# ThinkLib/Sail

Hardware: AMD Instinct MI355X
Metric: Msamples/s (paths x bounces) at 1920x1080 Cornell box (higher is better)
Workload: dtype f32; 1 GPU; cornell_box_readme_C2; width=1920, height=1080, bounces=8, spp=1024, launch_spp=1024, partition=tiles64x1, processes=one

## Files before the change

include/sail_hip.h:

```cpp
#ifndef SAIL_HIP_H
#define SAIL_HIP_H
#include <stddef.h>
#include <stdint.h>

#ifdef __cplusplus
extern "C" {
#endif

#define SAIL_ABI_VERSION 4

enum sail_status {
  SAIL_OK = 0,
  SAIL_E_INVALID = -1,
  SAIL_E_HIP = -2,
  SAIL_E_OOM = -3,
  SAIL_E_STATE = -4,
  SAIL_E_RCCL = -5,
  SAIL_E_NODEVICE = -6
};

enum sail_flags {
  SAIL_FLAG_AOV = 1u << 0,
  SAIL_FLAG_SEGMENT_COUNT = 1u << 1
};
// ... 133 lines not shown
  SAIL_JIT_MODE_FLAT = 0,
  SAIL_JIT_MODE_CULL = 1,
  SAIL_JIT_MODE_ROOM = 2
};
int sail_jit_compile(const sail_plugins* plugins, int mode, const int32_t* row_types, int rows, void* code,
                     size_t* bytes);
enum sail_kernel_jit_state {
  SAIL_KERNEL_JIT_NONE = 0,
  SAIL_KERNEL_JIT_PENDING = 1,
  SAIL_KERNEL_JIT_READY = 2,
  SAIL_KERNEL_JIT_FAILED = 3
};
typedef struct sail_kernel_info {
  char name[64];
  uint64_t build_id;
  int jit_state;
  int jit_from_cache;
  double jit_compile_ms;
  uint64_t jit_build_id;
  char jit_error[256];
} sail_kernel_info;
int sail_get_kernel_info(sail_ctx* ctx, sail_kernel_info* out);
int sail_kernel_ready(sail_ctx* ctx, int timeout_ms, int* ready);
int sail_set_jit_cache(const char* dir);
int sail_jit_prebuild(const float* objects, int n, const float* texparams, int tn, const float* lights, int ln,
                      const sail_plugins* plugins, const char* arch, const char* dir, int* built);

int sail_camera(const double eye[3], const double center[3], const double up[3], double fovy, double aspect,
                double znear, double zfar, double mvp_rowmajor[16]);
int sail_jitter_inverse(const double mvp_rowmajor[16], double jx, double jy, int width, int height, float inv_colmajor[16]);
int sail_schedule(const double mvp_rowmajor[16], int width, int height, int k0, int spp, float* inv_colmajor, float* seeds);

int sail_prim_bounds(const float* objects, int n, int tn, float* out_minmax);

int sail_comm_unique_id(char id[128]);
int sail_comm_init(sail_ctx* ctx, const char id[128], int nranks, int rank);
int sail_reduce(sail_ctx* ctx, int root);
int sail_accum_device_ptr(sail_ctx* ctx, void** ptr, size_t* bytes);
int sail_partition_tiles(int width, int height, int rank, int world, int* out_xywh, int capacity);
typedef struct sail_reduce_plan {
  int receives;
  int tiles;
  int aov_owner;
  int send_own_aovs;
  uint64_t samples;
} sail_reduce_plan;
int sail_plan_reduce(int width, int height, int rank, int world, int mode, uint64_t k, int root, sail_reduce_plan* out);
int sail_plan_keep(int width, int height, int rank, int world, int mode, const float* sums, float* out);
int sail_plan_load_part(uint64_t* missing, uint64_t* k, int parts, int part, uint64_t k_part);

int sail_math_probe(int fn, const float* x, const float* y, float* out, int count);
int sail_abi_version(void);
int sail_kernel_name(sail_ctx* ctx, char* name, int len);
int sail_filter_ms(sail_ctx* ctx, double* ms);

#ifdef __cplusplus
}
#endif
#endif
```

sail_amd/capi.py:

```python
from __future__ import annotations

import ctypes
import os
from typing import Optional, Sequence

import numpy as np

_HERE = os.path.dirname(os.path.abspath(__file__))
LIB_PATH = os.environ.get("SAIL_HIP_LIB") or os.path.join(_HERE, "lib", "libsail_hip.so")

SAIL_OK = 0
FLAG_AOV = 1
FLAG_SEGMENT_COUNT = 2
ACCUM_SUM, ACCUM_MIX, ACCUM_COMPAT8 = 0, 1, 2
PART_TILES, PART_SAMPLES = 0, 1
FILTER_COLOR, FILTER_GAMMA, FILTER_TONEMAPPING, FILTER_WINDOW = 0, 1, 2, 3
FILTER_WAVELET, FILTER_NORMAL, FILTER_POSITION = 4, 5, 6
DEBUG_CULL_MIN_PRIMS, DEBUG_FORCE_GENERIC, DEBUG_CULL_FMA, DEBUG_SAMPLE_GROUPS, DEBUG_FORCE_RCCL = 1, 2, 3, 4, 5
DEBUG_WAVEFRONT = 6
DEBUG_GROUP_ROUNDS = 7
DEBUG_CULL_GROUP_ROUNDS = 8
DEBUG_JIT = 9
DEBUG_JIT_WAIT = 10
DEBUG_JIT_NT = 12
DEBUG_JIT_NS = 11
KERNEL_JIT_NONE, KERNEL_JIT_PENDING, KERNEL_JIT_READY, KERNEL_JIT_FAILED = 0, 1, 2, 3
JIT_MODE_FLAT, JIT_MODE_CULL, JIT_MODE_ROOM = 0, 1, 2
DEBUG_DEFAULTS: dict = {}

EXPORTS = (
    "sail_create", "sail_create_multi", "sail_set_debug", "sail_destroy", "sail_last_error", "sail_device_count", "sail_device_info", "sail_set_scene",
    "sail_update_objects", "sail_set_accum_mode", "sail_set_partition", "sail_set_launch_samples",
    "sail_render", "sail_render_schedule", "sail_reset", "sail_sync", "sail_readback", "sail_read_accum",
    "sail_filter", "sail_get_stats", "sail_camera", "sail_jitter_inverse", "sail_schedule",
    "sail_comm_unique_id", "sail_comm_init", "sail_reduce", "sail_accum_device_ptr", "sail_partition_tiles",
    "sail_prim_bounds", "sail_math_probe", "sail_pick", "sail_kernel_name", "sail_filter_ms",
    "sail_abi_version", "sail_accum_parts", "sail_save_accum", "sail_load_accum", "sail_jit_compile",
    "sail_get_kernel_info", "sail_kernel_ready", "sail_set_jit_cache", "sail_jit_prebuild",
    "sail_plan_reduce", "sail_plan_keep", "sail_plan_load_part",
    "sail_noise_mark", "sail_noise_estimate", "sail_plan_until", "sail_render_until",
    "sail_denoise_defaults", "sail_denoise",
    "sail_temporal_defaults", "sail_gbuffer", "sail_temporal_begin", "sail_temporal_resolve", "sail_temporal_read",
    "sail_temporal_load_history",
)


class SailError(RuntimeError):
    pass


class Plugins(ctypes.Structure):
    _fields_ = [("shape_mask", ctypes.c_uint32), ("material_mask", ctypes.c_uint32),
                ("texture_mask", ctypes.c_uint32), ("light_mask", ctypes.c_uint32)]


class Stats(ctypes.Structure):
    _fields_ = [("samples", ctypes.c_uint64), ("segments", ctypes.c_uint64),
                ("nominal_segments", ctypes.c_uint64), ("kernel_ms", ctypes.c_double),
                ("last_launch_ms", ctypes.c_double), ("launches", ctypes.c_uint32)]


class KernelInfo(ctypes.Structure):
    _fields_ = [("name", ctypes.c_char * 64), ("build_id", ctypes.c_uint64), ("jit_state", ctypes.c_int),
                ("jit_from_cache", ctypes.c_int), ("jit_compile_ms", ctypes.c_double), ("jit_build_id", ctypes.c_uint64),
                ("jit_error", ctypes.c_char * 256)]


class ReducePlan(ctypes.Structure):
    _fields_ = [("receives", ctypes.c_int), ("tiles", ctypes.c_int), ("aov_owner", ctypes.c_int),
                ("send_own_aovs", ctypes.c_int), ("samples", ctypes.c_uint64)]


# ... 61 lines not shown
    vp = ctypes.c_void_p
    sig = {
        "sail_create": (ctypes.c_int, [ctypes.POINTER(vp), ctypes.c_int, ctypes.c_int, ctypes.c_int, ctypes.c_uint32]),
        "sail_create_multi": (ctypes.c_int, [ctypes.POINTER(vp), ctypes.c_int, ctypes.c_int, ctypes.POINTER(ctypes.c_int),
                                             ctypes.c_int, ctypes.c_uint32]),
        "sail_set_debug": (ctypes.c_int, [vp, ctypes.c_int, ctypes.c_int]),
        "sail_destroy": (None, [vp]),
        "sail_last_error": (ctypes.c_char_p, [vp]),
        "sail_device_count": (ctypes.c_int, [ctypes.POINTER(ctypes.c_int)]),
        "sail_device_info": (ctypes.c_int, [ctypes.c_int, ctypes.POINTER(ctypes.c_int), ctypes.POINTER(ctypes.c_int)]),
        "sail_set_scene": (ctypes.c_int, [vp, f32p, ctypes.c_int, f32p, ctypes.c_int, f32p, ctypes.c_int, ctypes.POINTER(Plugins)]),
        "sail_update_objects": (ctypes.c_int, [vp, f32p, ctypes.c_int]),
        "sail_set_accum_mode": (ctypes.c_int, [vp, ctypes.c_int]),
        "sail_set_partition": (ctypes.c_int, [vp, ctypes.c_int, ctypes.c_int, ctypes.c_int]),
        "sail_set_launch_samples": (ctypes.c_int, [vp, ctypes.c_int]),
        "sail_render": (ctypes.c_int, [vp, f32p, f32p, ctypes.c_float, ctypes.c_int]),
        "sail_render_schedule": (ctypes.c_int, [vp, f32p, f32p, f32p, ctypes.c_int, ctypes.c_int]),
        "sail_reset": (ctypes.c_int, [vp]),
        "sail_sync": (ctypes.c_int, [vp]),
        "sail_readback": (ctypes.c_int, [vp, f32p, f32p, f32p]),
        "sail_read_accum": (ctypes.c_int, [vp, f32p]),
        "sail_filter": (ctypes.c_int, [vp, ctypes.c_int, f32p, ctypes.c_float, ctypes.c_float, ctypes.c_float, f32p, ctypes.POINTER(ctypes.c_uint8)]),
        "sail_get_stats": (ctypes.c_int, [vp, ctypes.POINTER(Stats)]),
        "sail_camera": (ctypes.c_int, [f64p, f64p, f64p, ctypes.c_double, ctypes.c_double, ctypes.c_double, ctypes.c_double, f64p]),
        "sail_jitter_inverse": (ctypes.c_int, [f64p, ctypes.c_double, ctypes.c_double, ctypes.c_int, ctypes.c_int, f32p]),
        "sail_schedule": (ctypes.c_int, [f64p, ctypes.c_int, ctypes.c_int, ctypes.c_int, ctypes.c_int, f32p, f32p]),
        "sail_comm_unique_id": (ctypes.c_int, [ctypes.c_char_p]),
        "sail_comm_init": (ctypes.c_int, [vp, ctypes.c_char_p, ctypes.c_int, ctypes.c_int]),
        "sail_reduce": (ctypes.c_int, [vp, ctypes.c_int]),
        "sail_accum_device_ptr": (ctypes.c_int, [vp, ctypes.POINTER(vp), ctypes.POINTER(ctypes.c_size_t)]),
        "sail_partition_tiles": (ctypes.c_int, [ctypes.c_int, ctypes.c_int, ctypes.c_int, ctypes.c_int,
                                                 ctypes.POINTER(ctypes.c_int), ctypes.c_int]),
        "sail_prim_bounds": (ctypes.c_int, [f32p, ctypes.c_int, ctypes.c_int, f32p]),
        "sail_math_probe": (ctypes.c_int, [ctypes.c_int, f32p, f32p, f32p, ctypes.c_int]),
        "sail_abi_version": (ctypes.c_int, []),
        "sail_pick": (ctypes.c_int, [vp, f32p, ctypes.c_int, ctypes.POINTER(ctypes.c_int32), f32p]),
        "sail_kernel_name": (ctypes.c_int, [vp, ctypes.c_char_p, ctypes.c_int]),
        "sail_filter_ms": (ctypes.c_int, [vp, f64p]),
        "sail_accum_parts": (ctypes.c_int, [vp, ctypes.POINTER(ctypes.c_int)]),
        "sail_save_accum": (ctypes.c_int, [vp, ctypes.c_int, f32p, ctypes.POINTER(ctypes.c_uint64)]),
        "sail_load_accum": (ctypes.c_int, [vp, ctypes.c_int, f32p, ctypes.c_uint64]),
        "sail_jit_compile": (ctypes.c_int, [ctypes.POINTER(Plugins), ctypes.c_int, ctypes.POINTER(ctypes.c_int32), ctypes.c_int,
                                            vp, ctypes.POINTER(ctypes.c_size_t)]),
        "sail_get_kernel_info": (ctypes.c_int, [vp, ctypes.POINTER(KernelInfo)]),
        "sail_kernel_ready": (ctypes.c_int, [vp, ctypes.c_int, ctypes.POINTER(ctypes.c_int)]),
        "sail_set_jit_cache": (ctypes.c_int, [ctypes.c_char_p]),
        "sail_jit_prebuild": (ctypes.c_int, [f32p, ctypes.c_int, f32p, ctypes.c_int, f32p, ctypes.c_int, ctypes.POINTER(Plugins),
                                             ctypes.c_char_p, ctypes.c_char_p, ctypes.POINTER(ctypes.c_int)]),
        "sail_plan_reduce": (ctypes.c_int, [ctypes.c_int, ctypes.c_int, ctypes.c_int, ctypes.c_int, ctypes.c_int,
                                            ctypes.c_uint64, ctypes.c_int, ctypes.POINTER(ReducePlan)]),
        "sail_plan_keep": (ctypes.c_int, [ctypes.c_int, ctypes.c_int, ctypes.c_int, ctypes.c_int, ctypes.c_int, f32p, f32p]),
        "sail_plan_load_part": (ctypes.c_int, [ctypes.POINTER(ctypes.c_uint64), ctypes.POINTER(ctypes.c_uint64), ctypes.c_int,
                                               ctypes.c_int, ctypes.c_uint64]),
        "sail_noise_mark": (ctypes.c_int, [vp]),
        "sail_noise_estimate": (ctypes.c_int, [vp, ctypes.POINTER(NoiseInfo), f32p, f32p, ctypes.c_int]),
        "sail_plan_until": (ctypes.c_int, [ctypes.c_uint64, ctypes.c_uint64, ctypes.c_uint64, ctypes.POINTER(ctypes.c_uint64)]),
        "sail_render_until": (ctypes.c_int, [vp, f64p, f32p, ctypes.c_int, ctypes.c_double, ctypes.c_uint64, ctypes.c_uint64,
                                             ctypes.POINTER(NoiseInfo), ctypes.POINTER(ctypes.c_int),
                                             ctypes.POINTER(UntilStep), ctypes.c_int, ctypes.POINTER(ctypes.c_int)]),
        "sail_denoise_defaults": (ctypes.c_int, [ctypes.POINTER(DenoiseParams)]),
        "sail_denoise": (ctypes.c_int, [vp, ctypes.POINTER(DenoiseParams), f32p, f32p, ctypes.POINTER(ctypes.c_uint8),
                                        ctypes.POINTER(DenoiseInfo)]),
        "sail_temporal_defaults": (ctypes.c_int, [ctypes.POINTER(TemporalParams)]),
        "sail_gbuffer": (ctypes.c_int, [vp, f64p, f32p, f32p, ctypes.POINTER(ctypes.c_int32), f32p, f32p]),
        "sail_temporal_begin": (ctypes.c_int, [vp, f64p, f32p, ctypes.POINTER(TemporalParams), ctypes.POINTER(TemporalInfo)]),
        "sail_temporal_resolve": (ctypes.c_int, [vp, ctypes.POINTER(TemporalParams), f32p, ctypes.POINTER(ctypes.c_uint8),
# ... 135 lines not shown
    if rc:
        raise SailError(f"sail_temporal_defaults: {rc}")
    return {"cap": p.cap, "pos_tol": p.pos_tol, "display": p.display, "gamma_c": p.gamma_c}


def _temporal_params(params: Optional[dict], who: str):
    if params is None:
        return None
    d = temporal_defaults()
    unknown = set(params) - set(d)
    if unknown:
        raise SailError(f"{who}: unknown parameters {sorted(unknown)}")
    d.update(params)
    return TemporalParams(float(d["cap"]), float(d["pos_tol"]), int(d["display"]), float(d["gamma_c"]))


def _temporal_dict(i: TemporalInfo) -> dict:
    return {"k": int(i.k), "hit_pixels": int(i.hit_pixels), "history_pixels": int(i.history_pixels),
            "nonfinite": int(i.nonfinite), "kernel_ms": i.kernel_ms, "pass_ms": [i.pass_ms[j] for j in range(3)]}


def prim_bounds(objects, n: int, tn: int) -> np.ndarray:
    lib = load()
    rows = _f32(objects).reshape(-1)
    if rows.size < 18 * n:
        raise SailError("prim_bounds: fewer than 18 floats per row")
    out = np.zeros((max(n, 1), 6), dtype=np.float32)
    rc = lib.sail_prim_bounds(_ptr(rows), n, tn, _ptr(out))
    if rc:
        raise SailError(f"sail_prim_bounds: {rc}")
    return out[:n].reshape(n, 2, 3)


def math_probe(fn: int, x: np.ndarray, y: Optional[np.ndarray] = None) -> np.ndarray:
    lib = load()
    x = _f32(x)
    y = _f32(np.zeros_like(x) if y is None else y)
    out = np.zeros_like(x)
    rc = lib.sail_math_probe(fn, _ptr(x), _ptr(y), _ptr(out), int(x.size))
    if rc:
        raise SailError(f"sail_math_probe: {lib.sail_last_error(None).decode()}")
    return out


def device_count() -> int:
    lib = load()
    n = ctypes.c_int(0)
    lib.sail_device_count(ctypes.byref(n))
    return n.value


def device_info(device: int = 0):
    lib = load()
    cus, khz = ctypes.c_int(0), ctypes.c_int(0)
    if lib.sail_device_info(device, ctypes.byref(cus), ctypes.byref(khz)) != 0:
        raise SailError(f"sail_device_info({device}) failed")
    return cus.value, khz.value * 1e3


def set_jit_cache(path: Optional[str]):
    load().sail_set_jit_cache(None if path is None else path.encode())


def jit_prebuild(sc: dict, arch: str = "gfx950", cache_dir: Optional[str] = None) -> bool:
    lib = load()
    o, t, l = _f32(sc["objects"]), _f32(sc["texparams"]), _f32(sc["lights"])
# ... 313 lines not shown
```

sail_amd/csrc/sail_capi.cpp:

```cpp
#include <hip/hip_runtime.h>
#include <dlfcn.h>
#include <math.h>
#include <algorithm>
#include <cmath>
#include <stdarg.h>
#include <stdio.h>
#include <stdlib.h>
#include <string.h>
#include <string>
#include <vector>
#include "../../include/sail_hip.h"
#include "sail_device.h"

hipError_t sail_launch_trace(const SailTraceArgs& A, int blocks, hipStream_t s);
#include "sail_jit.h"
hipError_t sail_launch_filter(const SailFilterArgs& A, hipStream_t s);
hipError_t sail_launch_accum(const SailTraceArgs& A, int blocks, hipStream_t s);
hipError_t sail_launch_math(int fn, const float* x, const float* y, float* out, int count);
hipError_t sail_launch_sum(const SailSumArgs& A, hipStream_t s);
hipError_t sail_launch_negzero_unowned(float4* a, float4* b, int W, int H, int rank, int world, hipStream_t s);
hipError_t sail_launch_wavefront(const SailTraceArgs& A, const SailWfState& S, hipStream_t s);
hipError_t sail_launch_pick(const SailPrim* prims, int n, const float* rays, int count, int32_t* index, float* t,
                            hipStream_t s);
#include "sail_noise.h"
// ... 76 lines not shown
    out[2] = at(px, y);
  }
};

}

struct SceneBox { double lo[3], hi[3]; double diag; };

struct sail_ctx {
  int device = 0, W = 0, H = 0;
  uint32_t flags = 0;
  hipStream_t stream = nullptr;
  float4* accum = nullptr;
  float4* aovN = nullptr;
  float4* aovP = nullptr;
  float4* filterOut = nullptr;
  uint8_t* filterOut8 = nullptr;
  unsigned long long* segCounter = nullptr;
  SailPrim* prims = nullptr;
  float* tp = nullptr;
  float* lt = nullptr;
  int32_t* lightObjRow = nullptr;
  SailSample* samples = nullptr;
  int samplesCap = 0;
  int samplesPos = 0;
  SailSample* samplesPinned = nullptr;
  std::vector<SailSample> hostSamples;
  std::vector<float> objectsRows;
  std::vector<float> tpRows;
  int n = 0, tn = 0, ln = 0;
  sail_plugins plugins{};
  bool haveScene = false;
  int shadowAnyHit = 0;
  std::vector<unsigned long long> typeMasksHost;
  int cullMinPrims = 8;
  int lastGroups = 1;
  bool lastWavefront = false;
  int flatGroupRounds = 36;
  int cullGroupRounds = 64;
  int cullFma = 1;
  double primExtent = INFINITY;
  SceneBox scene{};
  int forceGeneric = 0;
  int forceGroups = 0;
  int wavefront = 0;
  int jit = 27;
  bool jitHave = false;
  SailJitSpec jitSpec;
  int jitMode = 0;
  int jitState = SAIL_KERNEL_JIT_NONE;
  SailJitKernel jitK;
  std::string jitError;
  int jitWait = 0;
  int jitNt = 0;
  int jitNs = 0;
  bool lastJit = false;
  int lastJitMode = 0;
  uint64_t lastBuildId = 0;
  std::vector<int> primTypes;
  float4* wf = nullptr;
  size_t wfSlots = 0;
  int numCUs = 256;
  float* stage = nullptr;
  size_t stageBytes = 0;
  int accumMode = SAIL_ACCUM_SUM;
  int rank = 0, world = 1, partMode = SAIL_PART_TILES;
// ... 375 lines not shown
}

double primExtent(const std::vector<SailPrim>& prims) {
  double m = 0.0;
  for (const SailPrim& p : prims)
    for (int k = 18; k < 24; k++) m = fmax(m, std::isfinite(p.a[k]) ? fabs((double)p.a[k]) : INFINITY);
  return m;
}

bool cullFmaOk(const sail_ctx* c) {
  const double e = fmax(fmax(fabs(c->eyeCache[0]), fabs(c->eyeCache[1])), fabs(c->eyeCache[2]));
  return c->cullFma && fmax(c->primExtent, e) < 4096.0;
}

int eyeNearScene(const sail_ctx* c) {
  double d2 = 0.0;
  for (int k = 0; k < 3; k++) {
    const double e = c->eyeCache[k];
    const double g = e < c->scene.lo[k] ? c->scene.lo[k] - e : (e > c->scene.hi[k] ? e - c->scene.hi[k] : 0.0);
    d2 += g * g;
  }
  return d2 == d2 && sqrt(d2) <= c->scene.diag;
}

void fillCats(std::vector<SailPrim>& prims, const float* texparams, int tn) {
  auto cat = [&](int row) {
    const int v = (tn > 0 && row >= 0 && row < tn) ? to_int(texparams[(size_t)row * 16]) : 0;
    return v < -1 ? -1 : (v > 32 ? 32 : v);
  };
  for (SailPrim& p : prims)
    p.cats = (int32_t)(((uint32_t)(uint16_t)(int16_t)cat(p.matRow)) | ((uint32_t)(uint16_t)(int16_t)cat(p.texRow) << 16));
}

void decodePrims(const float* objects, int n, int tn, uint32_t shapeMask, std::vector<SailPrim>& out, int* anyHitOk,
                 SceneBox* sbOut) {
  std::vector<PrimBox> raw((size_t)n);
  TexView o{objects, 18, n};
  const float L = 17.0f;
  out.assign((size_t)n, SailPrim{});
  *anyHitOk = 1;
  auto row = [&](float v) { return texel(gdiv(v, (float)(tn - 1)), tn); };
  for (int i = 0; i < n; i++) {
    const float rc = gdiv((float)i, (float)(n - 1));
    SailPrim& p = out[i];
    memset(&p, 0, sizeof p);
    const int cat = to_int(o.at(0.0f, rc));
    if (cat < 1 || cat > 9 || !((shapeMask >> cat) & 1u)) { p.type = 0; continue; }
    p.type = cat;
    float v3[3];
    switch (cat) {
      case SAIL_CUBE: case SAIL_RECTANGLE:
        o.readVec3(1.0f, rc, L, &p.a[0]); o.readVec3(4.0f, rc, L, &p.a[3]);
        p.rev = to_int(o.readFloat(7.0f, rc, L)) == 1;
        p.matRow = row(o.readFloat(8.0f, rc, L)); p.texRow = row(o.readFloat(9.0f, rc, L));
        o.readVec3(10.0f, rc, L, v3);
        if (cat == SAIL_RECTANGLE) rectFrameHost(p);
        break;
      case SAIL_SPHERE:
        o.readVec3(1.0f, rc, L, &p.a[0]); p.a[3] = o.readFloat(4.0f, rc, L);
        p.rev = to_int(o.readFloat(5.0f, rc, L)) == 1;
        p.matRow = row(o.readFloat(6.0f, rc, L)); p.texRow = row(o.readFloat(7.0f, rc, L));
        o.readVec3(8.0f, rc, L, v3);
        break;
      case SAIL_CONE: case SAIL_CYLINDER: case SAIL_DISK:
        o.readVec3(1.0f, rc, L, &p.a[0]); p.a[3] = o.readFloat(4.0f, rc, L); p.a[4] = o.readFloat(5.0f, rc, L);
        p.rev = to_int(o.readFloat(6.0f, rc, L)) == 1;
// ... 63 lines not shown
    src = c->samplesPinned + c->samplesPos;
  }
  c->samplesPos += count;
  HIPCHK(c, hipMemcpyAsync(dev, src, sizeof(SailSample) * count, hipMemcpyHostToDevice, c->stream));
  const long long px = ownedPixels(c);
  const long long stageStride = (long long)owned * 4096;
  const int stageSpp = (int)std::max<long long>(1, (long long)(kStageCapBytes / ((size_t)stageStride * 12)));
  const int L = launchSamples(c);
  for (int s0 = 0; s0 < count; s0 += L) {
    const int nspp = (count - s0) < L ? (count - s0) : L;
    SailTraceArgs A;
    memset(&A, 0, sizeof A);
    A.prims = c->prims; A.typeMasks = reinterpret_cast<const unsigned long long*>(c->prims + c->n);
    A.texparams = c->tp; A.lights = c->lt; A.lightObjRow = c->lightObjRow;
    A.samples = dev + s0;
    A.accum = c->accum; A.aovN = c->aovN; A.aovP = c->aovP; A.segCounter = c->segCounter;
    A.W = c->W; A.H = c->H; A.n = c->n; A.tn = c->tn; A.ln = c->ln;
    A.matMask = c->plugins.material_mask; A.texMask = c->plugins.texture_mask; A.lightMask = c->plugins.light_mask;
    A.maxBounces = maxBounces; A.spp = nspp; A.accumMode = c->accumMode;
    A.tilesX = tx; A.tilesY = ty;
    A.world = (c->partMode == SAIL_PART_SAMPLES) ? 1 : c->world;
    A.rank = (c->partMode == SAIL_PART_SAMPLES) ? 0 : c->rank;
    A.ownedTiles = owned;
    A.shadowAnyHit = c->shadowAnyHit;
    A.cullPrims = c->n >= c->cullMinPrims ? (cullFmaOk(c) ? 2 : 1) : 0;
    A.cullPrimary = eyeNearScene(c);
    A.kernelSet = kernelSetFor(c);
    memcpy(A.eye, c->eyeCache, sizeof A.eye);
    const bool wavefront = c->wavefront && A.kernelSet == SAIL_KSET_GENERIC && A.cullPrims;
    SailJitKernel jk;
    int jmode = 0;
    const bool jit = !wavefront && jitKernels(c, c->jitWait, &jk, &jmode);
    const int ns = jit ? c->jitSpec.ns : 1;
    int G = 1;
    if (c->forceGroups > 0) {
      G = c->forceGroups;
    } else if (A.kernelSet == SAIL_KSET_GENERIC && A.cullPrims) {
      const double rounds = (double)owned * 4.0 * ns / (double)(c->numCUs * 2);
      if (rounds < (double)c->cullGroupRounds) G = (int)ceil((double)c->cullGroupRounds / rounds);
    } else {
      const long long waves = (long long)owned * 16 * 4 * ns;
      const long long target = (long long)c->numCUs * 4 * 7 * c->flatGroupRounds;
      G = (int)((target + waves - 1) / waves);
      if (ns >= 16) G = 1;
    }
    if (G > nspp) G = nspp;
    if (G < 1) G = 1;
    if (nspp > stageSpp) G = 1;
    A.groupSpp = (nspp + G - 1) / G;
    if (ns > 1 && A.groupSpp < nspp && c->forceGroups <= 0) A.groupSpp = ((A.groupSpp + ns - 1) / ns) * ns;
    A.sampleGroups = (nspp + A.groupSpp - 1) / A.groupSpp;
    A.groupHome = (jit ? jmode == SAIL_JIT_MODE_ROOM : SAIL_GROUP_HOME_FOR(A.kernelSet)) ? 1 : 0;
    A.stageStride = stageStride;
    const bool staged = A.sampleGroups > 1;
    if (staged) {
      const size_t need = (size_t)A.stageStride * (size_t)nspp * 3 * sizeof(float);
      if (need > c->stageBytes) {
        if (c->stage) { HIPCHK(c, hipStreamSynchronize(c->stream)); HIPCHK(c, hipFree(c->stage)); c->stage = nullptr; }
        c->stageBytes = 0;
        if (hipMalloc(&c->stage, need) != hipSuccess) { c->stage = nullptr; return fail(c, SAIL_E_OOM, "sample-group stage"); }
        c->stageBytes = need;
      }
      A.stage = c->stage;
    }
    SailWfState WS;
    memset(&WS, 0, sizeof WS);
// ... 451 lines not shown
  if (n <= 0) return SAIL_OK;
  const size_t chunks = (size_t)(n + 63) / 64;
  c->typeMasksHost.assign(chunks * 16, 0ull);
  for (int i = 0; i < n; i++)
    if (prims[i].type >= 0 && prims[i].type < 16) c->typeMasksHost[(size_t)(i / 64) * 16 + prims[i].type] |= 1ull << (i % 64);
  HIPCHK(c, hipMemcpyAsync(c->prims, prims.data(), sizeof(SailPrim) * n, hipMemcpyHostToDevice, c->stream));
  HIPCHK(c, hipMemcpyAsync(c->prims + n, c->typeMasksHost.data(), chunks * 16 * sizeof(unsigned long long),
                           hipMemcpyHostToDevice, c->stream));
  return SAIL_OK;
}

int sail_set_scene(sail_ctx* c, const float* objects, int n, const float* texparams, int tn, const float* lights,
                   int ln, const sail_plugins* plugins) {
  if (!c) return SAIL_E_INVALID;
  if (!c->subs.empty()) {
    for (sail_ctx* s : c->subs)
      if (int rc = sail_set_scene(s, objects, n, texparams, tn, lights, ln, plugins)) return relay(c, rc, s);
    c->haveScene = true; c->n = n; c->tn = tn; c->ln = ln; c->dirty = false;
    c->loadMissing = 0;
    return SAIL_OK;
  }
  if (n < 0 || tn < 0 || ln < 0 || (n > 0 && !objects) || (tn > 0 && !texparams) || (ln > 0 && !lights) || !plugins)
    return fail(c, SAIL_E_INVALID, "sail_set_scene: bad arguments (n=%d tn=%d ln=%d)", n, tn, ln);
  if (n > 0 && tn < 1) return fail(c, SAIL_E_INVALID, "sail_set_scene: objects need texParams rows");
  HIPCHK(c, hipSetDevice(c->device));
  HIPCHK(c, hipStreamSynchronize(c->stream));
  c->plugins = *plugins;
  c->lastGroups = 1;
  c->lastWavefront = false;
  c->lastJit = false;
  std::vector<SailPrim> prims;
  decodePrims(objects, n, tn, plugins->shape_mask, prims, &c->shadowAnyHit, &c->scene);
  fillCats(prims, texparams, tn);
  c->primExtent = primExtent(prims);
  c->primTypes.clear();
  for (const SailPrim& q : prims) c->primTypes.push_back(q.type);
  std::vector<int32_t> lrow((size_t)(ln > 0 ? ln : 1), 0);
  TexView lv{lights, 18, ln};
  for (int r = 0; r < ln; r++) {
    const float rc = (ln == 1) ? NAN : gdiv((float)r, (float)(ln - 1));
    const int gi = to_int(lv.readFloat(1.0f, rc, 17.0f));
    lrow[r] = (n > 0) ? texel(gdiv((float)gi, (float)(n - 1)), n) : 0;
  }
  void* old[] = {c->prims, c->tp, c->lt, c->lightObjRow};
  for (void* b : old) if (b) HIPCHK(c, hipFree(b));
  c->prims = nullptr; c->tp = nullptr; c->lt = nullptr; c->lightObjRow = nullptr;
  const size_t pb = primBytes(n), tb = sizeof(float) * 16 * (size_t)(tn > 0 ? tn : 1),
               lb = sizeof(float) * 18 * (size_t)(ln > 0 ? ln : 1), rb = sizeof(int32_t) * lrow.size();
  if (hipMalloc(&c->prims, pb) != hipSuccess || hipMalloc(&c->tp, tb) != hipSuccess || hipMalloc(&c->lt, lb) != hipSuccess ||
      hipMalloc(&c->lightObjRow, rb) != hipSuccess)
    return fail(c, SAIL_E_OOM, "scene buffers");
  HIPCHK(c, hipMemsetAsync(c->tp, 0, tb, c->stream));
  HIPCHK(c, hipMemsetAsync(c->lt, 0, lb, c->stream));
  if (int rc = uploadPrims(c, prims)) return rc;
  if (tn > 0) HIPCHK(c, hipMemcpyAsync(c->tp, texparams, sizeof(float) * 16 * tn, hipMemcpyHostToDevice, c->stream));
  if (ln > 0) HIPCHK(c, hipMemcpyAsync(c->lt, lights, sizeof(float) * 18 * ln, hipMemcpyHostToDevice, c->stream));
  HIPCHK(c, hipMemcpyAsync(c->lightObjRow, lrow.data(), rb, hipMemcpyHostToDevice, c->stream));
  HIPCHK(c, hipStreamSynchronize(c->stream));
  c->objectsRows.assign(objects, objects + (size_t)n * 18);
  c->tpRows.assign(texparams, texparams + (size_t)tn * 16);
  c->n = n; c->tn = tn; c->ln = ln;
  c->haveScene = true;
  c->tpHaveCur = c->tpHavePrev = false;
  refreshJit(c);
  return resetAccum(c);
}

int sail_update_objects(sail_ctx* c, const float* objects, int n) {
  if (c && !c->subs.empty()) {
    for (sail_ctx* s : c->subs) if (int rc = sail_update_objects(s, objects, n)) return relay(c, rc, s);
    c->dirty = false;
    c->loadMissing = 0;
    return SAIL_OK;
  }
  if (!c || !c->haveScene) return c ? fail(c, SAIL_E_STATE, "sail_update_objects before sail_set_scene") : SAIL_E_INVALID;
  if (n != c->n || !objects) return fail(c, SAIL_E_INVALID, "sail_update_objects: n must stay %d", c->n);
  HIPCHK(c, hipSetDevice(c->device));
  std::vector<SailPrim> prims;
  decodePrims(objects, n, c->tn, c->plugins.shape_mask, prims, &c->shadowAnyHit, &c->scene);
  fillCats(prims, c->tpRows.data(), c->tn);
  c->primExtent = primExtent(prims);
  c->primTypes.clear();
  for (const SailPrim& q : prims) c->primTypes.push_back(q.type);
  HIPCHK(c, hipStreamSynchronize(c->stream));
  if (int rc = uploadPrims(c, prims)) return rc;
  HIPCHK(c, hipStreamSynchronize(c->stream));
  c->objectsRows.assign(objects, objects + (size_t)n * 18);
  c->tpHaveCur = c->tpHavePrev = false;
  refreshJit(c);
  return resetAccum(c);
}

int sail_set_accum_mode(sail_ctx* c, int mode) {
  if (!c) return SAIL_E_INVALID;
  if (mode < SAIL_ACCUM_SUM || mode > SAIL_ACCUM_COMPAT8) return fail(c, SAIL_E_INVALID, "accum mode %d", mode);
  if (!c->subs.empty()) {
    for (sail_ctx* s : c->subs) if (int rc = sail_set_accum_mode(s, mode)) return relay(c, rc, s);
    c->accumMode = mode; c->dirty = false;
    c->loadMissing = 0;
    return SAIL_OK;
  }
  if (mode != SAIL_ACCUM_SUM && c->partMode == SAIL_PART_SAMPLES && c->world > 1)
    return fail(c, SAIL_E_INVALID, "running-mean accumulation cannot be split by samples");
  HIPCHK(c, hipSetDevice(c->device));
  c->accumMode = mode;
  return resetAccum(c);
}

int sail_set_partition(sail_ctx* c, int rank, int world, int mode) {
  if (!c) return SAIL_E_INVALID;
  if (!c->subs.empty()) {
    if (rank != 0 || world != 1 || (mode != SAIL_PART_TILES && mode != SAIL_PART_SAMPLES))
      return fail(c, SAIL_E_INVALID, "multi-device context: partition must be (0, 1, mode), got (%d, %d, %d)", rank, world, mode);
// ... 972 lines not shown
  int anyHit = 0;
  decodePrims(objects, n, tn, plugins->shape_mask, prims, &anyHit, nullptr);
  for (const SailPrim& q : prims) t.primTypes.push_back(q.type);
  SailJitSpec spec;
  int mode = 0;
  if (built) *built = 0;
  if (!jitSpecFor(&t, &spec, &mode)) return SAIL_OK;
  std::string err;
  const bool cornell = mode == SAIL_JIT_MODE_FLAT && kernelSetFor(&t) == SAIL_KSET_CORNELL;
  for (int ns : {16, 1}) {
    if (cornell) spec.ns = ns;
    if (sail_jit_code_to_dir(arch, spec, dir, &err)) return fail(nullptr, SAIL_E_INVALID, "sail_jit_prebuild: %s", err.c_str());
    if (!cornell) break;
  }
  if (built) *built = 1;
  return SAIL_OK;
}

int sail_prim_bounds(const float* objects, int n, int tn, float* out) {
  if (n < 0 || (n > 0 && (!objects || !out))) return SAIL_E_INVALID;
  std::vector<SailPrim> prims;
  int anyHit = 0;
  decodePrims(objects, n, tn, ~0u, prims, &anyHit, nullptr);
  for (int i = 0; i < n; i++) {
    const SailPrim& p = prims[(size_t)i];
    for (int k = 0; k < 3; k++) {
      out[6 * i + k] = p.type ? p.a[18 + k] : INFINITY;
      out[6 * i + 3 + k] = p.type ? p.a[21 + k] : -INFINITY;
    }
  }
  return SAIL_OK;
}

int sail_partition_tiles(int width, int height, int rank, int world, int* out, int capacity) {
  if (width <= 0 || height <= 0 || world < 1 || rank < 0 || rank >= world || capacity < 0) return SAIL_E_INVALID;
  const int tx = (width + 63) / 64, ty = (height + 63) / 64;
  int count = 0;
  for (int t = rank; t < tx * ty; t += world) {
    if (out && count < capacity) {
      const int x0 = (t % tx) * 64, y0 = (t / tx) * 64;
      out[4 * count + 0] = x0;
      out[4 * count + 1] = y0;
      out[4 * count + 2] = (width - x0) < 64 ? (width - x0) : 64;
      out[4 * count + 3] = (height - y0) < 64 ? (height - y0) : 64;
    }
    count++;
  }
  return count;
}

int sail_plan_reduce(int width, int height, int rank, int world, int mode, uint64_t k, int root, sail_reduce_plan* out) {
  if (width <= 0 || height <= 0 || world < 1 || rank < 0 || rank >= world || root < 0 || root >= world || !out ||
      (mode != SAIL_PART_TILES && mode != SAIL_PART_SAMPLES))
    return fail(nullptr, SAIL_E_INVALID, "sail_plan_reduce: bad arguments");
  *out = planReduce(width, height, rank, world, mode, k, root);
  return SAIL_OK;
}

int sail_plan_keep(int width, int height, int rank, int world, int mode, const float* sums, float* out) {
  if (width <= 0 || height <= 0 || world < 1 || rank < 0 || rank >= world || !sums || !out ||
      (mode != SAIL_PART_TILES && mode != SAIL_PART_SAMPLES))
    return fail(nullptr, SAIL_E_INVALID, "sail_plan_keep: bad arguments");
  keepPart(width, height, rank, world, mode, sums, out);
  return SAIL_OK;
}

// ... 32 lines not shown
```

sail_amd/csrc/sail_device.h:

```cpp
#pragma once
#if defined(__HIPCC_RTC__)
using __hip_internal::int32_t;
using __hip_internal::int64_t;
using __hip_internal::uint8_t;
using __hip_internal::uint32_t;
using __hip_internal::uint64_t;
#else
#include <stdint.h>
#endif

enum {
  SAIL_CUBE = 1, SAIL_SPHERE = 2, SAIL_RECTANGLE = 3, SAIL_CONE = 4, SAIL_CYLINDER = 5, SAIL_DISK = 6,
  SAIL_HYPERBOLOID = 7, SAIL_PARABOLOID = 8, SAIL_CORNELLBOX = 9
};
enum { SAIL_AREA = 0, SAIL_POINT = 1, SAIL_SPOT = 2 };
enum { SAIL_MATTE = 1, SAIL_MIRROR = 2, SAIL_METAL = 3, SAIL_GLASS = 4 };
enum {
  SAIL_TEX_UNIFORM = 0, SAIL_TEX_CHECKERBOARD = 5, SAIL_TEX_CHECKERBOARD2 = 7, SAIL_TEX_BILERP = 8,
  SAIL_TEX_MIXF = 9, SAIL_TEX_SCALE = 10, SAIL_TEX_UVF = 11
};

struct __attribute__((aligned(16))) SailPrim {
  int32_t type;
  int32_t rev;
// ... 10 lines not shown
  float mixw;
  float pad[2];
};

struct SailTraceArgs {
  const SailPrim* prims;
  const unsigned long long* typeMasks;
  const float* texparams;
  const float* lights;
  const int32_t* lightObjRow;
  const SailSample* samples;
  float4* accum;
  float4* aovN;
  float4* aovP;
  unsigned long long* segCounter;
  float eye[3];
  int W, H;
  int n, tn, ln;
  uint32_t matMask, texMask, lightMask;
  int maxBounces;
  int spp;
  int accumMode;
  int tilesX, tilesY;
  int world, rank;
  int ownedTiles;
  int shadowAnyHit;
  int cullPrims;
  int cullPrimary;
  int kernelSet;
  int sampleGroups, groupSpp;
  int groupHome;
  float* stage;
  long long stageStride;
};

struct SailWfState {
  float4* o;
  float4* d;
  float4* f;
  float4* e;
  float4* s;
  float4* sp[6];
};

enum { SAIL_KSET_GENERIC = 0, SAIL_KSET_CORNELL = 1, SAIL_KSET_ROOM = 2 };
#define SAIL_GROUP_HOME_FOR(kernelSet) ((kernelSet) == SAIL_KSET_ROOM)
#define SAIL_SEG_SLOTS 64
#define SAIL_CULL_LDS_ROWS 72
#define SAIL_CULL_LDS_TP 136
#define SAIL_KSET_CORNELL_SHAPES ((1u << SAIL_CUBE) | (1u << SAIL_SPHERE) | (1u << SAIL_CORNELLBOX))
#define SAIL_KSET_CORNELL_MATS ((1u << SAIL_MATTE) | (1u << SAIL_MIRROR))
#define SAIL_KSET_CORNELL_TEX 0u
#define SAIL_KSET_CORNELL_LIGHTS 0u
#define SAIL_KSET_ROOM_SHAPES ((1u << SAIL_CUBE) | (1u << SAIL_SPHERE) | (1u << SAIL_RECTANGLE) | (1u << SAIL_CORNELLBOX))
#define SAIL_KSET_ROOM_MATS 0xffffffffu
#define SAIL_KSET_ROOM_TEX 0xffffffffu
#define SAIL_KSET_ROOM_LIGHTS 0xffffffffu

struct SailFilterArgs {
  const float4* accum;
  const float4* aovN;
  const float4* aovP;
  float4* out;
  uint8_t* out8;
  int W, H;
  int kind;
// ... 14 lines not shown
```

sail_amd/csrc/sail_trace.hip:

```cpp
#if !defined(__HIPCC_RTC__)
#include <hip/hip_runtime.h>
#include <stdint.h>
#endif
#include "sail_device.h"
#include "sail_math.h"
#include "sail_scan.h"

using namespace sm;


#define D __device__ __forceinline__

#if defined(SAIL_PHASE_TIMING) && SAIL_PHASE_TIMING
extern "C" __device__ unsigned long long g_sailPhase[12];
__device__ unsigned long long g_sailPhase[12];
#endif

namespace {

constexpr float kMaxDistance = 1e5f, kEps = 1e-5f, kOneMinusEps = 0.9999f, kInf = 1e5f;
constexpr float kPI = 3.141592653589793f, kInvPI = 0.3183098861837907f;
constexpr float kPiOver2 = 1.570796326794896f, kPiOver4 = 0.785398163397448f;

struct V3 { float x, y, z; };
// ... 1586 lines not shown
      Sweep sw;
      sw.best = kMaxDistance; sw.bi = -1; sw.bhl = v3s(0.0f);
      int key = 0;
      if constexpr (CULL) segsW += (unsigned long long)__popcll(__builtin_amdgcn_ballot_w64(alive));
      if (alive) {
        if constexpr (!CULL) segs++;
        sw = sweepRay(c, ray, depth == 1);
        if (sw.best >= kMaxDistance) {
          if (depth == 1 && aovs && k + pixel / kPX == A.spp - 1) {
            const size_t g = (size_t)homeY(pixel) * A.W + homeX(pixel);
            const V3 qn = v3s(0.0f) / 2.0f + 0.5f, qp = normalize(v3s(0.0f));
            if (A.aovN) A.aovN[g] = make_float4(qn.x, qn.y, qn.z, 1.0f);
            if (A.aovP) A.aovP[g] = make_float4(qp.x, qp.y, qp.z, 1.0f);
          }
          alive = false;
        } else if (byPrim) {
          key = 1 + sw.bi;
          if constexpr (FAM && !CULL && kCornellRow >= 0) {
            if (sw.bi == kCornellRow) {
              const SailPrim& cp = PRIM(c, kCornellRow);
              const V3 h = ray.o + sw.best * ray.d, mn = P3(cp, 0), mx = P3(cp, 3);
              const int face = h.x < mn.x + 0.0001f ? 0 : h.x > mx.x - 0.0001f ? 1 : h.y < mn.y + 0.0001f ? 2
                             : h.y > mx.y - 0.0001f ? 3 : h.z < mn.z + 0.0001f ? 4 : 5;
              key = 1 + kRows + face;
            }
          }
        } else {
          const SailPrim& p = PRIM(c, sw.bi);
          int mc = matCat(p);
          mc = (mc >= 0 && mc < 5) ? mc : 0;
          key = 1 + mc * 10 + p.type;
        }
      }
      PHASE_MARK(pc, 0);
      int rank = 0;
      int nAlive;
      auto dropState = [&]() {
        ray.o = v3s(0.0f); ray.d = v3s(0.0f); ray.rx = ray.ry = ray.rz = 0.0f;
        fpdf = v3s(0.0f); sw.best = 0.0f; sw.bi = 0; pixel = 0;
      };
      auto scatterTo = [&](int d) {
        if constexpr (kPack == 2) {
          sSt4[0][d] = make_float4(ray.o.x, ray.o.y, ray.o.z, ray.d.x);
          sSt4[1][d] = make_float4(ray.d.y, ray.d.z, fpdf.x, fpdf.y);
          sSt4[2][d] = make_float4(fpdf.z, sw.best, __int_as_float(pixel | (sw.bi << 10)), __int_as_float(key));
        } else {
          sSt2[0][d] = make_float2(ray.o.x, ray.o.y); sSt2[1][d] = make_float2(ray.o.z, ray.d.x);
          sSt2[2][d] = make_float2(ray.d.y, ray.d.z); sSt2[3][d] = make_float2(fpdf.x, fpdf.y);
          sSt2[4][d] = make_float2(fpdf.z, sw.best);
          sSt2[5][d] = make_float2(__int_as_float(pixel | (sw.bi << 10)), __int_as_float(key));
        }
      };
      const bool sortNow = kSort1 || depth > 1;
      if (sortNow) {
      if constexpr (twoBar) {
      if (alive) rank = atomicAdd(&sCnt2[ph][key], 1);
      PHASE_MARK(pc, 7);
      __syncthreads();
      PHASE_MARK(pc, 8);
      {
        const int v = sCnt2[ph][lane];
        const int incl = waveScanIncl(v);
        nAlive = __builtin_amdgcn_readlane(incl, 63);
        const int start = __shfl(incl - v, key, 64);
        if (alive) scatterTo(start + rank);
        dropState();
      }
      PHASE_MARK(pc, 9);
      __syncthreads();
      PHASE_MARK(pc, 10);
      if (wave == 0) sCnt2[ph][lane] = 0;
      ph ^= 1;
      } else {
      int* const sCnt = sCnt2[0];
      if (alive) rank = atomicAdd(&sCnt[key], 1);
      PHASE_MARK(pc, 7);
      __syncthreads();
      PHASE_MARK(pc, 8);
      if (wave == 0) {
        const int v = sCnt[lane];
        const int incl = waveScanIncl(v);
        sStart[lane] = incl - v;
        if (lane == 63) sStart[kKeys] = incl;
        sCnt[lane] = 0;
      }
      PHASE_MARK(pc, 9);
// ... 630 lines not shown
```

Measured before the change: 101,000 Msamples/s.

## Retire non-emissive matte hits early on the last bounce and skip sort

Adds a host-side analysis that marks primitives whose emission is zero and whose matte BRDF is finite. On the final bounce, lanes hitting such primitives are retired before shading, and the binning sort is skipped when every primitive qualifies. This removes shading and sort work whose result cannot contribute radiance. It adds scene-dependent branching and a per-context plan, and it only applies to non-culled, non-family kernels.

```diff
diff --git a/include/sail_hip.h b/include/sail_hip.h
--- a/include/sail_hip.h
+++ b/include/sail_hip.h
@@ -189,6 +189,8 @@
 int sail_schedule(const double mvp_rowmajor[16], int width, int height, int k0, int spp, float* inv_colmajor, float* seeds);
 
 int sail_prim_bounds(const float* objects, int n, int tn, float* out_minmax);
+int sail_plan_last_bounce(const float* objects, int n, const float* texparams, int tn, const sail_plugins* plugins,
+                          int kernel_lights, uint32_t* quiet_rows, int* skip_sort);
 
 int sail_comm_unique_id(char id[128]);
 int sail_comm_init(sail_ctx* ctx, const char id[128], int nranks, int rank);
diff --git a/sail_amd/capi.py b/sail_amd/capi.py
--- a/sail_amd/capi.py
+++ b/sail_amd/capi.py
@@ -37,7 +37,7 @@
     "sail_prim_bounds", "sail_math_probe", "sail_pick", "sail_kernel_name", "sail_filter_ms",
     "sail_abi_version", "sail_accum_parts", "sail_save_accum", "sail_load_accum", "sail_jit_compile",
     "sail_get_kernel_info", "sail_kernel_ready", "sail_set_jit_cache", "sail_jit_prebuild",
-    "sail_plan_reduce", "sail_plan_keep", "sail_plan_load_part",
+    "sail_plan_reduce", "sail_plan_keep", "sail_plan_load_part", "sail_plan_last_bounce",
     "sail_noise_mark", "sail_noise_estimate", "sail_plan_until", "sail_render_until",
     "sail_denoise_defaults", "sail_denoise",
     "sail_temporal_defaults", "sail_gbuffer", "sail_temporal_begin", "sail_temporal_resolve", "sail_temporal_read",
@@ -165,6 +165,8 @@
         "sail_partition_tiles": (ctypes.c_int, [ctypes.c_int, ctypes.c_int, ctypes.c_int, ctypes.c_int,
                                                  ctypes.POINTER(ctypes.c_int), ctypes.c_int]),
         "sail_prim_bounds": (ctypes.c_int, [f32p, ctypes.c_int, ctypes.c_int, f32p]),
+        "sail_plan_last_bounce": (ctypes.c_int, [f32p, ctypes.c_int, f32p, ctypes.c_int, ctypes.POINTER(Plugins), ctypes.c_int,
+                                                 ctypes.POINTER(ctypes.c_uint32), ctypes.POINTER(ctypes.c_int)]),
         "sail_math_probe": (ctypes.c_int, [ctypes.c_int, f32p, f32p, f32p, ctypes.c_int]),
         "sail_abi_version": (ctypes.c_int, []),
         "sail_pick": (ctypes.c_int, [vp, f32p, ctypes.c_int, ctypes.POINTER(ctypes.c_int32), f32p]),
@@ -366,6 +368,18 @@
     return out[:n].reshape(n, 2, 3)
 
 
+def plan_last_bounce(sc: dict, kernel_lights: bool):
+    lib = load()
+    o, t = _f32(sc["objects"]), _f32(sc["texparams"])
+    pl = Plugins(*[int(m) for m in plugin_masks(sc["plugins"])])
+    quiet, skip = ctypes.c_uint32(0), ctypes.c_int(0)
+    rc = lib.sail_plan_last_bounce(_ptr(o), sc["n"], _ptr(t), sc["tn"], ctypes.byref(pl), int(bool(kernel_lights)),
+                                   ctypes.byref(quiet), ctypes.byref(skip))
+    if rc:
+        raise SailError(f"sail_plan_last_bounce: {rc}: {lib.sail_last_error(None).decode()}")
+    return int(quiet.value), int(skip.value)
+
+
 def math_probe(fn: int, x: np.ndarray, y: Optional[np.ndarray] = None) -> np.ndarray:
     lib = load()
     x = _f32(x)
diff --git a/sail_amd/csrc/sail_capi.cpp b/sail_amd/csrc/sail_capi.cpp
--- a/sail_amd/csrc/sail_capi.cpp
+++ b/sail_amd/csrc/sail_capi.cpp
@@ -132,6 +132,8 @@
   sail_plugins plugins{};
   bool haveScene = false;
   int shadowAnyHit = 0;
+  uint32_t lastQuietRows[2] = {0u, 0u};
+  int lastSkipSort[2] = {0, 0};
   std::vector<unsigned long long> typeMasksHost;
   int cullMinPrims = 8;
   int lastGroups = 1;
@@ -573,6 +575,53 @@
     p.cats = (int32_t)(((uint32_t)(uint16_t)(int16_t)cat(p.matRow)) | ((uint32_t)(uint16_t)(int16_t)cat(p.texRow) << 16));
 }
 
+void lastBounceRows(const std::vector<SailPrim>& prims, const float* tp, int tn, uint32_t matMask, bool lights,
+                    uint32_t* quietRows, int* skipSort) {
+  *quietRows = 0;
+  *skipSort = 0;
+  const int n = (int)prims.size();
+  if (n < 1 || n > 32 || tn < 1 || !tp) return;
+  constexpr float kEps = 1e-5f, kInvPI = 0.3183098861837907f;
+  bool skip = true, any = false;
+  for (int i = 0; i < n; i++) {
+    const SailPrim& p = prims[(size_t)i];
+    if (p.type == 0) continue;
+    any = true;
+    uint32_t eb[3];
+    memcpy(eb, p.em, sizeof eb);
+    const bool emPosZero = (eb[0] | eb[1] | eb[2]) == 0u;
+    const bool emBlack = p.em[0] == 0.0f && p.em[1] == 0.0f && p.em[2] == 0.0f;
+    const bool matte = (int)(short)(p.cats & 0xffff) == SAIL_MATTE;
+    bool matteOk = true;
+    if (matte) {
+      const bool rowsOk = p.matRow >= 0 && p.matRow < tn && p.texRow >= 0 && p.texRow < tn;
+      if (lights || !rowsOk) {
+        matteOk = false;
+      } else if ((matMask >> SAIL_MATTE) & 1u) {
+        const float kd = tp[(size_t)p.matRow * 16 + 1], sigma = tp[(size_t)p.matRow * 16 + 2];
+        float sc[4][3] = {{0.25f, 0.75f, 0.25f}, {0.25f, 0.25f, 0.75f}, {1.0f, 1.0f, 1.0f}, {0.0f, 0.0f, 0.0f}};
+        int ncol = 0;
+        if (p.type == SAIL_CORNELLBOX) {
+          ncol = 4;
+        } else if ((p.cats >> 16) == SAIL_TEX_UNIFORM) {
+          for (int k = 0; k < 3; k++) sc[0][k] = tp[(size_t)p.texRow * 16 + 1 + k];
+          ncol = 1;
+        }
+        matteOk = sigma < kEps && ncol > 0;
+        for (int q = 0; q < ncol; q++)
+          for (int k = 0; k < 3; k++) {
+            volatile float f = kd * sc[q][k];
+            f = f * kInvPI;
+            if (!std::isfinite((float)f)) matteOk = false;
+          }
+      }
+    }
+    if (emPosZero && matteOk) *quietRows |= 1u << i;
+    else if (!(matteOk && !emBlack)) skip = false;
+  }
+  *skipSort = (any && skip) ? 1 : 0;
+}
+
 void decodePrims(const float* objects, int n, int tn, uint32_t shapeMask, std::vector<SailPrim>& out, int* anyHitOk,
                  SceneBox* sbOut) {
   std::vector<PrimBox> raw((size_t)n);
@@ -702,6 +751,11 @@
     int jmode = 0;
     const bool jit = !wavefront && jitKernels(c, c->jitWait, &jk, &jmode);
     const int ns = jit ? c->jitSpec.ns : 1;
+    {
+      const bool kl = jit ? c->jitSpec.kl != 0u : A.kernelSet != SAIL_KSET_CORNELL;
+      A.lastQuietRows = A.cullPrims ? 0u : c->lastQuietRows[kl];
+      A.lastSkipSort = A.cullPrims ? 0 : c->lastSkipSort[kl];
+    }
     int G = 1;
     if (c->forceGroups > 0) {
       G = c->forceGroups;
@@ -1219,6 +1273,8 @@
   std::vector<SailPrim> prims;
   decodePrims(objects, n, tn, plugins->shape_mask, prims, &c->shadowAnyHit, &c->scene);
   fillCats(prims, texparams, tn);
+  for (int l = 0; l < 2; l++)
+    lastBounceRows(prims, texparams, tn, plugins->material_mask, l != 0, &c->lastQuietRows[l], &c->lastSkipSort[l]);
   c->primExtent = primExtent(prims);
   c->primTypes.clear();
   for (const SailPrim& q : prims) c->primTypes.push_back(q.type);
@@ -1266,6 +1322,9 @@
   std::vector<SailPrim> prims;
   decodePrims(objects, n, c->tn, c->plugins.shape_mask, prims, &c->shadowAnyHit, &c->scene);
   fillCats(prims, c->tpRows.data(), c->tn);
+  for (int l = 0; l < 2; l++)
+    lastBounceRows(prims, c->tpRows.data(), c->tn, c->plugins.material_mask, l != 0, &c->lastQuietRows[l],
+                   &c->lastSkipSort[l]);
   c->primExtent = primExtent(prims);
   c->primTypes.clear();
   for (const SailPrim& q : prims) c->primTypes.push_back(q.type);
@@ -2304,6 +2363,19 @@
   return SAIL_OK;
 }
 
+int sail_plan_last_bounce(const float* objects, int n, const float* texparams, int tn, const sail_plugins* plugins,
+                          int kernel_lights, uint32_t* quiet_rows, int* skip_sort) {
+  if (n < 0 || tn < 0 || (n > 0 && !objects) || (tn > 0 && !texparams) || !plugins || !quiet_rows || !skip_sort ||
+      (n > 0 && tn < 1))
+    return fail(nullptr, SAIL_E_INVALID, "sail_plan_last_bounce: bad arguments");
+  std::vector<SailPrim> prims;
+  int anyHit = 0;
+  decodePrims(objects, n, tn, plugins->shape_mask, prims, &anyHit, nullptr);
+  fillCats(prims, texparams, tn);
+  lastBounceRows(prims, texparams, tn, plugins->material_mask, kernel_lights != 0, quiet_rows, skip_sort);
+  return SAIL_OK;
+}
+
 int sail_partition_tiles(int width, int height, int rank, int world, int* out, int capacity) {
   if (width <= 0 || height <= 0 || world < 1 || rank < 0 || rank >= world || capacity < 0) return SAIL_E_INVALID;
   const int tx = (width + 63) / 64, ty = (height + 63) / 64;
diff --git a/sail_amd/csrc/sail_device.h b/sail_amd/csrc/sail_device.h
--- a/sail_amd/csrc/sail_device.h
+++ b/sail_amd/csrc/sail_device.h
@@ -66,6 +66,8 @@
   int groupHome;
   float* stage;
   long long stageStride;
+  uint32_t lastQuietRows;
+  int lastSkipSort;
 };
 
 struct SailWfState {
diff --git a/sail_amd/csrc/sail_trace.hip b/sail_amd/csrc/sail_trace.hip
--- a/sail_amd/csrc/sail_trace.hip
+++ b/sail_amd/csrc/sail_trace.hip
@@ -1642,6 +1642,16 @@
           key = 1 + mc * 10 + p.type;
         }
       }
+      const bool lastB = !CULL && !FAM && depth == A.maxBounces;
+      if constexpr (!CULL && !FAM) {
+        if (lastB) __builtin_amdgcn_s_setprio(0);
+        if (lastB && alive && ((A.lastQuietRows >> (sw.bi & 31)) & 1u) != 0u &&
+            !(depth == 1 && aovs && k + pixel / kPX == A.spp - 1)) {
+          E_STORE(pixel, E_LOAD(pixel) + v3s(0.0f) * fpdf);
+          alive = false;
+          key = 0;
+        }
+      }
       PHASE_MARK(pc, 0);
       int rank = 0;
       int nAlive;
@@ -1661,7 +1671,7 @@
           sSt2[5][d] = make_float2(__int_as_float(pixel | (sw.bi << 10)), __int_as_float(key));
         }
       };
-      const bool sortNow = kSort1 || depth > 1;
+      const bool sortNow = (kSort1 || depth > 1) && !(lastB && A.lastSkipSort != 0);
       if (sortNow) {
       if constexpr (twoBar) {
       if (alive) rank = atomicAdd(&sCnt2[ph][key], 1);
```

Measured after the change: 104,300 Msamples/s (median of 6 runs). +3.3%, better.
